# lmangani/duckdb-fastlane

Measured on AMD Instinct MI355X. Metric: decoded values/sec (lineitem_full SF100 full scan), higher is better.
Workload: dtype u8..u64 integer unpack -> int32/int64/string_t

## Files before the change

duckdb-fastlane_amd/csrc/fls_decode.hip:

```cpp
#include <hip/hip_runtime.h>

#include <algorithm>
#include <cstdlib>
#include <cstring>
#include <map>
#include <mutex>
#include <tuple>

#include "fls_alp.hpp"
#include "fls_decode.hpp"
#include "fls_format.hpp"
#include "fls_unpack.hpp"

#include "fls_decode_dev.hpp"

namespace fls {
using namespace dec;
namespace {

#ifndef FLS_WAVES_PER_SIMD
#define FLS_WAVES_PER_SIMD 4
#endif
template <bool RATING>
__global__ __launch_bounds__(256, FLS_WAVES_PER_SIMD) void decode_kernel(const DevChunk *__restrict__ chunks, uint32_t nchunks,
                                                        uint32_t *__restrict__ err, uint32_t p_bytes,
                                                        uint32_t v_bytes, uint32_t *__restrict__ queue,
                                                        const uint32_t *__restrict__ split, uint32_t npieces,
                                                        uint32_t flags) {
    extern __shared__ __attribute__((aligned(16))) uint8_t lds_raw[];
    const uint32_t shared_queue = flags & 1u, prio = (flags >> 1) & 3u;
    if (prio == 1) __builtin_amdgcn_s_setprio(1);
    else if (prio == 2) __builtin_amdgcn_s_setprio(2);
    else if (prio == 3) __builtin_amdgcn_s_setprio(3);
    const uint32_t w = uni(threadIdx.x >> 6);
    const uint32_t lp = (uint32_t)(size_t)((lu8 *)lds_raw + w * (p_bytes + v_bytes));
    const uint32_t lv = lp + p_bytes;
    const uint32_t stride = shared_queue ? 0u : gridDim.x * kWaves, first = blockIdx.x * kWaves + w;
    if (split && shared_queue) {
        const FLS_GLOBAL uint32_t *sp = gptr(split);
        const uint32_t nst = flags >> 8;
        for (;;) {
            uint32_t q = 0;
            if (__lane_id() == 0) q = atomicAdd(queue, 1u);
            q = uni(q);
            if (q >= nst + npieces) break;
            const uint32_t i = q < nst ? q : q + 1;
            decode_range(chunks, nchunks, uni(sp[i]), uni(sp[i + 1]), lp, lv, v_bytes, err);
        }
        return;
    }
    if (split) {
        const FLS_GLOBAL uint32_t *sp = gptr(split);
        decode_range(chunks, nchunks, uni(sp[first]), uni(sp[first + 1]), lp, lv, v_bytes, err);
        if (!queue) return;
        const FLS_GLOBAL uint32_t *pp = sp + stride + 1;
        for (;;) {
            uint32_t p = 0;
            if (__lane_id() == 0) p = atomicAdd(queue, 1u);
            p = uni(p);
            if (p >= npieces) break;
            decode_range(chunks, nchunks, uni(pp[p]), uni(pp[p + 1]), lp, lv, v_bytes, err);
        }
        return;
    }
    for (uint32_t ci = next_chunk(queue, UINT32_MAX, first, stride); ci < nchunks;
         ci = next_chunk(queue, ci, first, stride)) {
        const uint32_t nvec = gptr(chunks)[ci].nvec;
        if (nvec == 0) continue;
        decode_chunk(chunks + ci, lp, lv, v_bytes, err, nvec << 8);
    }
}

}

#ifdef FLS_WAVE_TRACE
extern "C" int fls_trace_reset(void) {
    const uint32_t z = 0;
    return hipMemcpyToSymbol(HIP_SYMBOL(g_trace_n), &z, sizeof(z)) == hipSuccess ? 0 : -1;
}
extern "C" int64_t fls_trace_read(void *dst, uint32_t cap) {
    uint32_t n = 0;
    if (hipDeviceSynchronize() != hipSuccess ||
        hipMemcpyFromSymbol(&n, HIP_SYMBOL(g_trace_n), sizeof(n)) != hipSuccess)
        return -1;
    const uint32_t k = std::min(std::min(n, cap), kTraceCap);
    if (k && hipMemcpyFromSymbol(dst, HIP_SYMBOL(g_trace), (size_t)k * sizeof(TraceRec)) != hipSuccess) return -1;
    return n;
}
#endif

namespace {
std::mutex g_occ_mu;
std::map<int, int> g_cus;
std::map<std::tuple<int, const void *, int, size_t>, int> g_occ;
}

int device_cus() {
    int dev = 0, cus = 256;
    if (hipGetDevice(&dev) != hipSuccess) return 256;
    {
        std::lock_guard<std::mutex> lk(g_occ_mu);
        if (auto it = g_cus.find(dev); it != g_cus.end()) return it->second;
    }
    if (hipDeviceGetAttribute(&cus, hipDeviceAttributeMultiprocessorCount, dev) != hipSuccess) return 256;
    std::lock_guard<std::mutex> lk(g_occ_mu);
    g_cus[dev] = cus;
    return cus;
}

int occupancy(const void *kernel, int block, size_t shmem) {
    int dev = 0, per_cu = 1;
    if (hipGetDevice(&dev) != hipSuccess) return 1;
    const auto key = std::make_tuple(dev, kernel, block, shmem);
    {
        std::lock_guard<std::mutex> lk(g_occ_mu);
        if (auto it = g_occ.find(key); it != g_occ.end()) return it->second;
    }
    if (hipOccupancyMaxActiveBlocksPerMultiprocessor(&per_cu, kernel, block, shmem) != hipSuccess) return 1;
    std::lock_guard<std::mutex> lk(g_occ_mu);
    g_occ[key] = per_cu;
    return per_cu;
}

int decode_grid_size(uint32_t shmem_per_block) {
    const int cus = device_cus();
    int per_cu = occupancy(reinterpret_cast<const void *>(decode_kernel<false>), 64 * kWaves, shmem_per_block);
    if (const char *e = getenv("FLS_BLOCKS_PER_CU")) per_cu = std::min(per_cu, std::max(1, atoi(e)));
    return cus * std::max(1, per_cu);
}

uint32_t decode_waves(const DecodeGeom &geom) {
    const uint32_t shmem = kWaves * (geom.p_bytes + geom.v_bytes);
    return (uint32_t)(geom.grid > 0 ? geom.grid : decode_grid_size(shmem)) * kWaves;
}

static inline uint64_t vec_cost(const DevChunk &d) { return 1024ull * d.ob + 128ull * d.max_w + 512; }

SplitPlan balanced_split(const DevChunk *h, uint32_t n, uint32_t nw, uint32_t static_pct, uint32_t pieces_per_wave,
                         std::vector<uint32_t> &pos) {
    uint64_t total = 0, nvecs = 0;
    for (uint32_t i = 0; i < n; ++i) {
        total += h[i].nvec * vec_cost(h[i]);
        nvecs += h[i].nvec;
    }
    SplitPlan plan;
    plan.waves = (uint32_t)std::min<uint64_t>(nw, (nvecs + kWaves - 1) / kWaves * kWaves);
    if (plan.waves == 0) plan.waves = kWaves;
    static_pct = std::min(static_pct, 100u);
    plan.pieces = static_pct < 100 ? plan.waves * std::max(1u, pieces_per_wave) : 0;
    const uint64_t stat = (uint64_t)((unsigned __int128)total * static_pct / 100);
    pos.clear();
    pos.reserve(plan.positions());
    uint64_t acc = 0;
    uint32_t i = 0;
    auto at = [&](uint64_t tgt) {
        while (i < n && acc + h[i].nvec * vec_cost(h[i]) <= tgt) {
            acc += h[i].nvec * vec_cost(h[i]);
            ++i;
        }
        pos.push_back(i < n ? (i << 7 | (uint32_t)((tgt - acc) / vec_cost(h[i]))) : n << 7);
    };
    for (uint32_t w = 0; w <= plan.waves; ++w) at((uint64_t)((unsigned __int128)stat * w / plan.waves));
    at(stat);
    for (uint32_t p = 1; p < plan.pieces; ++p) at(stat + (uint64_t)((unsigned __int128)(total - stat) * p / plan.pieces));
    if (plan.pieces) pos.push_back(n << 7);
    return plan;
}

SplitPlan guided_split(const DevChunk *h, uint32_t n, uint32_t nw, uint32_t factor, uint32_t min_vecs,
                       std::vector<uint32_t> &pos) {
    uint64_t total = 0;
    for (uint32_t i = 0; i < n; ++i) total += h[i].nvec * vec_cost(h[i]);
    factor = std::max(1u, factor);
    min_vecs = std::max(1u, min_vecs);
    nw = std::max<uint32_t>(nw, kWaves);
    std::vector<uint32_t> b;
    b.reserve(n + n / 4);
    uint64_t acc = 0;
    for (uint32_t i = 0; i < n; ++i) {
        const uint32_t nv = h[i].nvec;
        if (nv == 0) continue;
        const uint64_t vc = vec_cost(h[i]), cc = nv * vc;
        const uint64_t target = std::max<uint64_t>((total - acc) / ((uint64_t)factor * nw), (uint64_t)min_vecs * vc);
        uint32_t parts = 1;
        if (cc > target)
            parts = (uint32_t)std::min<uint64_t>((cc + target - 1) / target, (nv + min_vecs - 1) / min_vecs);
        for (uint32_t p = 0; p < parts; ++p) b.push_back(i << 7 | (uint32_t)((uint64_t)nv * p / parts));
        acc += cc;
    }
    const uint32_t items = (uint32_t)b.size();
    b.push_back(n << 7);
    SplitPlan plan;
    plan.guided = true;
    plan.waves = std::min<uint32_t>(nw, std::max<uint32_t>(kWaves, (items + kWaves - 1) / kWaves * kWaves));
    plan.pieces = items > plan.waves ? items - plan.waves : 0;
    pos.clear();
    pos.reserve(plan.positions());
    for (uint32_t w = 0; w <= plan.waves; ++w) pos.push_back(b[std::min(w, items)]);
    for (uint32_t p = 0; p <= plan.pieces; ++p) pos.push_back(b[std::min(plan.waves + p, items)]);
    return plan;
}

hipError_t launch_decode(const DevChunk *d_chunks, uint32_t nchunks, uint32_t *d_err, const DecodeGeom &geom,
                         hipStream_t stream, uint32_t *d_queue, const uint32_t *d_split, SplitPlan plan,
                         bool shared_queue, int prio) {
    if (nchunks == 0) return hipSuccess;
    const uint32_t shmem = kWaves * (geom.p_bytes + geom.v_bytes);
    int grid;
    if (d_split && shared_queue) {
        grid = std::min<int>(geom.grid > 0 ? geom.grid : decode_grid_size(shmem), (int)(plan.waves / kWaves));
    } else if (d_split) {
        grid = (int)(plan.waves / kWaves);
        if (!plan.pieces) d_queue = nullptr;
    } else {
        grid = std::min<int>(geom.grid > 0 ? geom.grid : decode_grid_size(shmem), (nchunks + kWaves - 1) / kWaves);
    }
    if (d_queue && !shared_queue) {
        const hipError_t e = hipMemsetAsync(d_queue, 0, sizeof(uint32_t), stream);
        if (e != hipSuccess) return e;
    }
    hipLaunchKernelGGL(rating_launch() ? decode_kernel<true> : decode_kernel<false>, dim3(grid), dim3(64 * kWaves), shmem,
                       stream, d_chunks, nchunks, d_err,
                       geom.p_bytes, geom.v_bytes, d_queue, d_split, plan.pieces,
                       (uint32_t)(shared_queue && d_queue) | (uint32_t)(prio & 3) << 1 |
                           (d_split && shared_queue ? plan.waves << 8 : 0u));
    return hipGetLastError();
}

bool &rating_launch() {
    static thread_local bool f = false;
    return f;
}

namespace {
__global__ __launch_bounds__(64) void probe_regions_kernel(const ProbeRegion *__restrict__ r, uint32_t n) {
    const uint32_t lane = threadIdx.x;
    for (uint32_t i = blockIdx.x; i < n; i += gridDim.x) {
        const uint64_t p = (uint64_t)r[i].out, nb = r[i].bytes >> 10;
        FLS_GLOBAL v4u *o = (FLS_GLOBAL v4u *)((uint64_t)uni((uint32_t)(p >> 32)) << 32 | (uint64_t)uni((uint32_t)p));
        const v4u z = {0u, 0u, 0u, 0u};
        for (uint64_t b = 0; b < nb; ++b) o[b * 64 + lane] = z;
    }
}
__global__ __launch_bounds__(256) void probe_fill_kernel(v4u *__restrict__ out) {
    ((FLS_GLOBAL v4u *)out)[(size_t)blockIdx.x * 256 + threadIdx.x] = v4u{0u, 0u, 0u, 0u};
}
}

hipError_t probe_placement(const ProbeRegion *d_regions, uint32_t nregions, uint8_t *const *bufs,
                           const uint64_t *buf_bytes, uint32_t nbuf, int reps, hipStream_t stream, float *chunk_ms,
                           float *fill_ms) {
    int dev = 0, cus = 256;
    hipError_t e = hipGetDevice(&dev);
    if (e != hipSuccess) return e;
    if (hipDeviceGetAttribute(&cus, hipDeviceAttributeMultiprocessorCount, dev) != hipSuccess) cus = 256;
    hipEvent_t a, b;
    if ((e = hipEventCreate(&a)) != hipSuccess) return e;
    if ((e = hipEventCreate(&b)) != hipSuccess) {
        hipEventDestroy(a);
        return e;
    }
    float best_c = 1e30f, best_f = 1e30f;
    for (int r = 0; r <= reps && e == hipSuccess; ++r) {
        float ms = 0;
        hipEventRecord(a, stream);
        hipLaunchKernelGGL(probe_regions_kernel, dim3(cus * 16), dim3(64), 0, stream, d_regions, nregions);
        hipEventRecord(b, stream);
        if ((e = hipEventSynchronize(b)) != hipSuccess) break;
        hipEventElapsedTime(&ms, a, b);
        if (r) best_c = std::min(best_c, ms);
        hipEventRecord(a, stream);
        for (uint32_t i = 0; i < nbuf; ++i)
            if (buf_bytes[i] >= 4096)
                hipLaunchKernelGGL(probe_fill_kernel, dim3((uint32_t)(buf_bytes[i] >> 12)), dim3(256), 0, stream,
                                   (v4u *)bufs[i]);
        hipEventRecord(b, stream);
        if ((e = hipEventSynchronize(b)) != hipSuccess) break;
// ... 13 lines not shown
```

duckdb-fastlane_amd/csrc/fls_decode.hpp:

```cpp
#pragma once
#include <hip/hip_runtime.h>

#include <cstdint>
#include <vector>

namespace fls {

struct DevChunk {
    const uint8_t *chunk;
    const uint8_t *dict;
    uint8_t *out;
    uint32_t nvec;
    uint32_t dict_count;
    uint32_t meta_off;
    uint32_t packed_off;
    uint32_t aux_off;
    uint8_t enc, T, vbits, ob;
    uint64_t heap_host;
    uint32_t heap_bytes;
    union {
        uint32_t vec_base;
        uint32_t max_w;
    };
};
static_assert(sizeof(DevChunk) == 64, "DevChunk is 64 B");

enum : uint32_t { KERR_DICT_CODE = 1, KERR_RUN_INDEX = 2, KERR_BAD_DESC = 4, KERR_FSST = 8 };
enum : uint32_t { KERR_LDS_BASE = 32 };

struct DecodeGeom {
    uint32_t p_bytes = 256, v_bytes = 0;
    int grid = 0;
};

struct SplitPlan {
    uint32_t waves = 0, pieces = 0;
    bool guided = false;
    size_t positions() const { return waves ? (size_t)waves + pieces + 2 : 0; }
};

hipError_t launch_decode(const DevChunk *d_chunks, uint32_t nchunks, uint32_t *d_err, const DecodeGeom &geom,
                         hipStream_t stream, uint32_t *d_queue = nullptr, const uint32_t *d_split = nullptr,
                         SplitPlan plan = SplitPlan(), bool shared_queue = false, int prio = 0);
uint32_t decode_waves(const DecodeGeom &geom);
SplitPlan balanced_split(const DevChunk *h, uint32_t n, uint32_t nw, uint32_t static_pct, uint32_t pieces_per_wave,
                         std::vector<uint32_t> &pos);
SplitPlan guided_split(const DevChunk *h, uint32_t n, uint32_t nw, uint32_t factor, uint32_t min_vecs,
                       std::vector<uint32_t> &pos);
enum : int {
    kFsstPlain = 1, kFsstTwoQ = 2, kFsstZeroFlush = 4, kFsstW6 = 8, kFsstCirc = 16, kFsstLenFromSym = 32, kFsstAbsLds = 64, kFsstEarlyGather = 128,
    kFsstDefault = kFsstW6 | kFsstZeroFlush | kFsstAbsLds,
    kFsstSegSparse = kFsstPlain,
    kFsstSegPackedLen = kFsstLenFromSym,
    kFsstSegWide = kFsstCirc,
    kFsstSegDouble = kFsstEarlyGather,
    kFsstSegBatch = 256,
    kFsstAblateRecords = 512, kFsstAblateFlush = 1024, kFsstAblateWrite = 2048,
    kFsstSegLean = 4096,
    kFsstSegD8 = 8192,
    kFsstSegLazy = 16384,
    kFsstSegW4 = 32768
};
struct FsstLaunch {
    int bytes_per_lane = 8;
    bool small = false;
    uint32_t *queue = nullptr;
    bool reset_queue = true;
    int waves_per_cu = 0;
    int grid_cus = 0;
    int variant = kFsstDefault;
    bool seg = false;
    int seg_cap = 4096;
};
hipError_t launch_fsst(const DevChunk *d_chunks, uint32_t nchunks, uint32_t nvecs, uint32_t *d_err,
                       hipStream_t stream, const FsstLaunch &how);
struct FusedLaunch {
    uint32_t fsst_per16 = 6;
    uint32_t piece = 2;
    bool halving = false;
    uint32_t fsst_static_pct = 0;
    bool static_first = true;
    int waves_per_cu = 0;
    int x = 0;
    uint32_t tail_chunks = 0, tail_split = 1;
};
hipError_t launch_fused(const DevChunk *d_main, uint32_t nmain, const DevChunk *d_fsst, uint32_t nfsst,
                        uint32_t nfvecs, bool small, uint32_t *d_err, const DecodeGeom &geom, hipStream_t stream,
                        uint32_t *d_queues, const FusedLaunch &how);
bool fsst_variant_built(int variant, bool seg, int bytes_per_lane);
bool fused_x_built(int x);
hipError_t launch_fsst_sp(const DevChunk *d_chunks, uint32_t nchunks, uint32_t nvecs, uint32_t *d_err,
                          hipStream_t stream);
struct DictVec {
    const uint8_t *packed;
    const uint8_t *tab;
    uint8_t *out;
    uint32_t base;
    uint32_t info;
};
static_assert(sizeof(DictVec) == 32, "DictVec is 32 B");
constexpr uint32_t kDictWgMaxEntries = 64;
inline bool dictstr_eligible(const DevChunk &c) {
    return c.enc == 3  && c.ob == 16 && c.T == 32 && c.nvec > 0 && c.dict_count >= 1 &&
           c.dict_count <= kDictWgMaxEntries && c.dict && ((uintptr_t)c.dict & 15) == 0 && ((uintptr_t)c.out & 15) == 0 &&
           (((uintptr_t)c.chunk + c.packed_off) & 15) == 0;
}
hipError_t launch_dictstr(const DictVec *d_vecs, uint32_t nvecs, uint32_t *d_err, hipStream_t stream);
int decode_grid_size(uint32_t shmem_per_block);
int device_cus();
int occupancy(const void *kernel, int block, size_t shmem);

bool &rating_launch();

struct ProbeRegion {
    uint8_t *out;
    uint64_t bytes;
};
hipError_t probe_placement(const ProbeRegion *d_regions, uint32_t nregions, uint8_t *const *bufs,
                           const uint64_t *buf_bytes, uint32_t nbuf, int reps, hipStream_t stream, float *chunk_ms,
                           float *fill_ms);
inline void chunk_lds_need(uint8_t enc, uint8_t T, uint8_t ob, uint32_t dict_count, uint32_t max_w,
                           uint32_t &p_bytes, uint32_t &v_bytes) {
    p_bytes = 128 * max_w + 128;
    v_bytes = 0;
    if (enc == 2  && T < 64) v_bytes = 128 * T;
    if (enc == 4 ) v_bytes = 2048;
    if (enc == 3 ) {
        const uint32_t d = dict_count * ob;
        v_bytes = 4096 + (d <= 4096 ? ((d + 15) & ~15u) : 0);
    }
}

}
```

duckdb-fastlane_amd/csrc/fls_decode_dev.hpp:

```cpp
#pragma once
#include <hip/hip_runtime.h>

#include <algorithm>
#include <cstdlib>
#include <cstring>

#include "fls_alp.hpp"
#include "fls_decode.hpp"
#include "fls_format.hpp"
#include "fls_unpack.hpp"

namespace fls {
namespace dec {
namespace {
using namespace dev;

constexpr int kWaves = 4;

using gv4 = const FLS_GLOBAL v4u;
using gu8 = const FLS_GLOBAL uint8_t;
using ov4 = FLS_GLOBAL v4u;
using ou8 = FLS_GLOBAL uint8_t;
using lv4 = FLS_LDS v4u;
using lu8 = FLS_LDS uint8_t;
// ... 437 lines not shown
template <>
struct AlpScale<32> {
    float fm, im;
    __device__ __forceinline__ AlpScale(uint32_t e, uint32_t f) : fm(kF10F[f]), im(kIF10F[e]) {}
    __device__ __forceinline__ uint32_t one(uint32_t d) const {
        return __float_as_uint((float)(int32_t)d * fm * im);
    }
    __device__ __forceinline__ v4u apply(v4u x) const { return mk4(one(x.x), one(x.y), one(x.z), one(x.w)); }
};

template <int T_>
struct PathAlp {
    static constexpr int T = T_;
    static constexpr uint32_t kMaxE = T_ == 64 ? kAlpMaxExpD : kAlpMaxExpF;
    using Aux = NoAux;
    gu8 *aux_base;
    uint32_t *err;
    __device__ __forceinline__ PathAlp(const DevChunk &c, const Lds &, uint32_t, uint32_t *e)
        : aux_base(gptr(c.chunk) + c.aux_off), err(e) {}
    __device__ __forceinline__ gu8 *aux_ptr(const DevChunk &, const VecInfo &) const { return nullptr; }
    template <bool FULL>
    __device__ __forceinline__ void vec(const Lds &s, const VecInfo &x, const Aux &, ou8 *out, uint32_t lane) const {
        const uint32_t exc = x.acount & 0xFFFF;
        const uint32_t e = min((x.acount >> 16) & 0xFF, kMaxE), f = min(x.acount >> 24, e);
        const AlpScale<T> sc(e, f);
        const uint32_t limit = x.nvals * (T / 8);
#pragma unroll
        for (uint32_t j = 0; j < T / 8; ++j) {
            const uint32_t ci = lane + 64 * j;
            const v4u v = sc.apply(add_base<T>(unpack_chunk<T>(s.P, x.W, ci), x.base));
            if (FULL) st16(out, 16 * ci, v);
            else store16<T / 8>(out, 16 * ci, limit, v);
            seq();
        }
        if (exc == 0) return;
        __builtin_amdgcn_s_waitcnt(0x0F70);
        gu8 *ea = aux_base + x.aoff;
        const FLS_GLOBAL uint16_t *pos = reinterpret_cast<const FLS_GLOBAL uint16_t *>(ea);
        gu8 *val = ea + ((2 * exc + 15) & ~15u);
        bool bad = false;
        for (uint32_t k = lane; k < exc; k += 64) {
            const uint32_t p = pos[k];
            if (p >= x.nvals) { bad = true; continue; }
            if (T == 64) {
                reinterpret_cast<FLS_GLOBAL uint64_t *>(out)[p] = reinterpret_cast<const FLS_GLOBAL uint64_t *>(val)[k];
            } else {
                reinterpret_cast<FLS_GLOBAL uint32_t *>(out)[p] = reinterpret_cast<const FLS_GLOBAL uint32_t *>(val)[k];
            }
        }
        if (bad) atomicOr(err, KERR_BAD_DESC);
    }
};

template <class Path, int L>
__device__ __attribute__((noinline)) void run_chunk(const DevChunk *chunk_generic, uint32_t lds_p, uint32_t lds_v,
                                                    uint32_t v_bytes, uint32_t *err_generic, uint32_t vrange) {
    const uint64_t cp = (uint64_t)chunk_generic;
    const FLS_GLOBAL DevChunk *cptr =
        (const FLS_GLOBAL DevChunk *)((uint64_t)uni((uint32_t)(cp >> 32)) << 32 | uni((uint32_t)cp));
    DevChunk c;
    {
        const FLS_GLOBAL v4u *q = reinterpret_cast<const FLS_GLOBAL v4u *>(cptr);
        v4u *d = reinterpret_cast<v4u *>(&c);
        d[0] = q[0];
        d[1] = q[1];
        d[2] = q[2];
        d[3] = q[3];
    }
    Lds s;
    s.P = (lv4 *)(size_t)uni(lds_p);
    s.V = (lu8 *)(size_t)uni(lds_v);
    s.v_bytes = uni(v_bytes);
    const uint64_t ep = (uint64_t)err_generic;
    uint32_t *err = (uint32_t *)((uint64_t)uni((uint32_t)(ep >> 32)) << 32 | uni((uint32_t)ep));
    const uint32_t lane = __lane_id();
    const Path path(c, s, lane, err);
    using Aux = typename Path::Aux;
    const uint32_t nvec = c.nvec;
    const uint32_t ob = c.ob;
    const ChunkMetas m = load_metas(c, lane);
    gv4 *packed = reinterpret_cast<gv4 *>(gptr(c.chunk) + c.packed_off);
    gv4 *dummy = reinterpret_cast<gv4 *>(gptr(c.chunk));
    ou8 *out = gptr(c.out);
    const uint32_t vb = uni(vrange) & 0xFF, ve = min(uni(vrange) >> 8, nvec);
    const uint32_t last_nvals = rl(m.nvbw, nvec - 1) & 0xFFFF;
    const uint32_t nfull = (ve == nvec && last_nvals != kVectorSize) ? ve - 1 : ve;

#ifdef FLS_PREFETCH2
    if (vb < ve) {
        v4u ra[L], rb[L];
        VecInfo xa = vec_info(m, vb);
        Aux aa, ab;
        aa.load(path.aux_ptr(c, xa), lane);
        prefetch<L, true>(packed + xa.poff16, 8 * xa.W, dummy, lane, ra);
        VecInfo xb = vec_info(m, min(vb + 1, ve - 1));
        ab.load(path.aux_ptr(c, xb), lane);
        prefetch<L, true>(packed + xb.poff16, 8 * xb.W, dummy, lane, rb);
        uint32_t v = vb;
        for (;;) {
            if (v >= nfull) break;
            wave_sync();
            stage<L>(s.P, ra, 8 * xa.W, lane);
            {
                const VecInfo xn = vec_info(m, min(v + 2, ve - 1));
                Aux an;
                an.load(path.aux_ptr(c, xn), lane);
                prefetch<L, true>(packed + xn.poff16, 8 * xn.W, dummy, lane, ra);
                wave_sync();
                path.template vec<true>(s, xa, aa, out + (size_t)v * kVectorSize * ob, lane);
                xa = xn;
                aa = an;
            }
            ++v;
            if (v >= nfull) break;
            wave_sync();
            stage<L>(s.P, rb, 8 * xb.W, lane);
            {
                const VecInfo xn = vec_info(m, min(v + 2, ve - 1));
                Aux an;
                an.load(path.aux_ptr(c, xn), lane);
                prefetch<L, true>(packed + xn.poff16, 8 * xn.W, dummy, lane, rb);
                wave_sync();
                path.template vec<true>(s, xb, ab, out + (size_t)v * kVectorSize * ob, lane);
                xb = xn;
                ab = an;
            }
            ++v;
        }
        if (nfull < ve) {
            wave_sync();
            const bool in_a = ((v - vb) & 1) == 0;
            if (in_a) stage<L>(s.P, ra, 8 * xa.W, lane);
            else stage<L>(s.P, rb, 8 * xb.W, lane);
            wave_sync();
            if (in_a) path.template vec<false>(s, xa, aa, out + (size_t)v * kVectorSize * ob, lane);
            else path.template vec<false>(s, xb, ab, out + (size_t)v * kVectorSize * ob, lane);
        }
    }
    return;
#endif
    v4u r[L];
    Aux aux, aux_next;
    VecInfo cur = vec_info(m, vb);
    aux.load(path.aux_ptr(c, cur), lane);
    prefetch<L>(packed + cur.poff16, 8 * cur.W, dummy, lane, r);
    uint32_t v = vb;
    if (vb < nfull) {
        stage<L>(s.P, r, 8 * cur.W, lane);
        VecInfo nxt = vec_info(m, vb + 1 < ve ? vb + 1 : vb);
        aux_next.load(path.aux_ptr(c, nxt), lane);
        prefetch<L>(packed + nxt.poff16, 8 * nxt.W, dummy, lane, r);
        wave_sync();
        path.template vec<true>(s, cur, aux, out + (size_t)vb * kVectorSize * ob, lane);
        cur = nxt;
        aux = aux_next;
        for (v = vb + 1; v < nfull; ++v) {
            wave_sync();
            stage<L>(s.P, r, 8 * cur.W, lane);
            nxt = vec_info(m, v + 1 < ve ? v + 1 : v);
            aux_next.load(path.aux_ptr(c, nxt), lane);
            prefetch<L>(packed + nxt.poff16, 8 * nxt.W, dummy, lane, r);
            wave_sync();
            path.template vec<true>(s, cur, aux, out + (size_t)v * kVectorSize * ob, lane);
            cur = nxt;
            aux = aux_next;
        }
    }
    if (nfull < ve) {
        wave_sync();
        stage<L>(s.P, r, 8 * cur.W, lane);
        wave_sync();
        path.template vec<false>(s, cur, aux, out + (size_t)v * kVectorSize * ob, lane);
    }
}

template <class Path, int L>
__device__ __forceinline__ void call_l(const DevChunk *c, uint32_t lp, uint32_t lv, uint32_t vb, uint32_t *err,
                                       uint32_t max_w, uint32_t vr) {
    if constexpr (L > 1) {
        if (max_w <= 4 * L) {
            call_l<Path, L / 2>(c, lp, lv, vb, err, max_w, vr);
            return;
        }
    }
    run_chunk<Path, L>(c, lp, lv, vb, err, vr);
}
template <class Path>
__device__ __forceinline__ void call(const DevChunk *c, uint32_t lp, uint32_t lv, uint32_t vb, uint32_t *err,
                                     uint32_t max_w, uint32_t vr) {
    call_l<Path, Path::T / 8>(c, lp, lv, vb, err, max_w, vr);
}

template <int OB>
__device__ __forceinline__ void call_dict(const DevChunk *c, uint32_t lp, uint32_t lv, uint32_t vb, uint32_t *err,
                                          uint32_t dict_count, uint32_t max_w, uint32_t vr) {
    if (dict_count * OB + 4096 <= vb) call<PathDict<OB, true>>(c, lp, lv, vb, err, max_w, vr);
    else call<PathDict<OB, false>>(c, lp, lv, vb, err, max_w, vr);
}

__device__ __forceinline__ uint32_t next_chunk(uint32_t *queue, uint32_t prev, uint32_t first, uint32_t stride) {
    if (prev == UINT32_MAX && stride) return first;
    if (!queue) return prev + stride;
    uint32_t ci = 0;
    if (__lane_id() == 0) ci = atomicAdd(queue, 1u);
    return stride + uni(ci);
}

#ifdef FLS_WAVE_TRACE
struct TraceRec {
    uint64_t t0, t1;
    uint32_t wave, vr, hw_id, xcc_id, shape, max_w;
};
constexpr uint32_t kTraceCap = 1u << 20;
__device__ TraceRec g_trace[kTraceCap];
__device__ uint32_t g_trace_n;
#endif

__device__ __forceinline__ void decode_chunk_body(const DevChunk *cg, uint32_t lp, uint32_t lv, uint32_t v_bytes,
                                                  uint32_t *err, uint32_t vr);
__device__ __forceinline__ void decode_chunk(const DevChunk *cg, uint32_t lp, uint32_t lv, uint32_t v_bytes,
                                             uint32_t *err, uint32_t vr) {
#ifdef FLS_WAVE_TRACE
    const uint64_t t0 = wall_clock64();
    decode_chunk_body(cg, lp, lv, v_bytes, err, vr);
    const uint64_t t1 = wall_clock64();
    if (__lane_id() == 0) {
        const uint32_t i = atomicAdd(&g_trace_n, 1u);
        if (i < kTraceCap) {
            const FLS_GLOBAL DevChunk *c = gptr(cg);
            TraceRec &r = g_trace[i];
            r.t0 = t0;
            r.t1 = t1;
            r.wave = blockIdx.x * kWaves + (threadIdx.x >> 6);
            r.vr = vr;
            r.hw_id = __builtin_amdgcn_s_getreg((31 << 11) | 4);
// ... 5 lines not shown
#else
    decode_chunk_body(cg, lp, lv, v_bytes, err, vr);
#endif
}
__device__ __forceinline__ void decode_chunk_body(const DevChunk *cg, uint32_t lp, uint32_t lv, uint32_t v_bytes,
                                                  uint32_t *err, uint32_t vr) {
    const FLS_GLOBAL DevChunk *c = gptr(cg);
    const uint32_t dc = c->dict_count, mw = c->max_w;
    const uint32_t enc = c->enc, T = c->T, ob = c->ob;
    switch (enc) {
    case ENC_FFOR:
        switch (T) {
        case 64: call<PathFfor<64>>(cg, lp, lv, v_bytes, err, mw, vr); break;
        case 32: call<PathFfor<32>>(cg, lp, lv, v_bytes, err, mw, vr); break;
        case 16: call<PathFfor<16>>(cg, lp, lv, v_bytes, err, mw, vr); break;
        default: call<PathFfor<8>>(cg, lp, lv, v_bytes, err, mw, vr); break;
        }
        break;
    case ENC_DELTA:
        switch (T) {
        case 64: call<PathDelta64>(cg, lp, lv, v_bytes, err, mw, vr); break;
        case 32: call<PathDeltaSmall<32>>(cg, lp, lv, v_bytes, err, mw, vr); break;
        case 16: call<PathDeltaSmall<16>>(cg, lp, lv, v_bytes, err, mw, vr); break;
        default: call<PathDeltaSmall<8>>(cg, lp, lv, v_bytes, err, mw, vr); break;
        }
        break;
    case ENC_DICT:
        switch (ob) {
        case 16: call_dict<16>(cg, lp, lv, v_bytes, err, dc, mw, vr); break;
        case 8: call_dict<8>(cg, lp, lv, v_bytes, err, dc, mw, vr); break;
        case 4: call_dict<4>(cg, lp, lv, v_bytes, err, dc, mw, vr); break;
        case 2: call_dict<2>(cg, lp, lv, v_bytes, err, dc, mw, vr); break;
        default: call_dict<1>(cg, lp, lv, v_bytes, err, dc, mw, vr); break;
        }
        break;
    case ENC_ALP:
        if (T == 64) call<PathAlp<64>>(cg, lp, lv, v_bytes, err, mw, vr);
        else call<PathAlp<32>>(cg, lp, lv, v_bytes, err, mw, vr);
        break;
    case ENC_RLE:
        switch (ob) {
        case 8: call<PathRle<8>>(cg, lp, lv, v_bytes, err, mw, vr); break;
        case 4: call<PathRle<4>>(cg, lp, lv, v_bytes, err, mw, vr); break;
        case 2: call<PathRle<2>>(cg, lp, lv, v_bytes, err, mw, vr); break;
        default: call<PathRle<1>>(cg, lp, lv, v_bytes, err, mw, vr); break;
        }
        break;
    default:
        if ((threadIdx.x & 63) == 0) atomicOr(err, KERR_BAD_DESC);
        break;
    }
}

__device__ __forceinline__ void decode_range(const DevChunk *chunks, uint32_t nchunks, uint32_t s0, uint32_t s1,
                                             uint32_t lp, uint32_t lv, uint32_t v_bytes, uint32_t *err) {
    const uint32_t ce = min(s1 >> 7, nchunks), vend = s1 & 127;
    uint32_t vb = s0 & 127;
    for (uint32_t ci = s0 >> 7; ci < ce || (ci == ce && ci < nchunks && vb < vend); ++ci, vb = 0) {
        const uint32_t nvec = gptr(chunks)[ci].nvec;
        const uint32_t ve = min(ci == ce ? vend : nvec, nvec);
        if (vb < ve) decode_chunk(chunks + ci, lp, lv, v_bytes, err, vb | ve << 8);
    }
}

}
}
}
```

duckdb-fastlane_amd/csrc/fls_fsst.hip:

```cpp
#include <hip/hip_runtime.h>

#include <algorithm>
#include <cstdio>
#include <cstdlib>

#include "fls_decode.hpp"
#include "fls_decode_dev.hpp"
#include "fls_format.hpp"
#include "fls_unpack.hpp"

namespace fls {
namespace {
using namespace dev;

using gv4 = const FLS_GLOBAL v4u;
using gu8 = const FLS_GLOBAL uint8_t;
using ov4 = FLS_GLOBAL v4u;
using lv4 = FLS_LDS v4u;
using lu8 = FLS_LDS uint8_t;
using lu16 = FLS_LDS uint16_t;
using lu32 = FLS_LDS uint32_t;
using lu64 = FLS_LDS uint64_t;

__device__ __forceinline__ uint32_t rl(uint32_t x, uint32_t l) { return __builtin_amdgcn_readlane(x, l); }
// ... 951 lines not shown
    const uint32_t shmem = K == Kind::Seg ? SegLds<SMALL, X>::kWave : CpLds<SMALL>::kWave;
    auto kern = fsst_kernel<K, SMALL, QUEUE, X>;
    static const bool lds_at_zero = [kern] {
        hipFuncAttributes a{};
        return hipFuncGetAttributes(&a, reinterpret_cast<const void *>(kern)) == hipSuccess && a.sharedSizeBytes == 0;
    }();
    if (!lds_at_zero) {
        fprintf(stderr, "fsst_kernel: static LDS present or attributes unavailable; cannot address LDS from 0\n");
        return hipErrorInvalidDeviceFunction;
    }
    int cus = device_cus(), per_cu = occupancy(reinterpret_cast<const void *>(kern), 64, shmem);
    if (how.grid_cus > 0) cus = std::min(cus, how.grid_cus);
    const int full = cus * std::max(1, per_cu);
    int wpc = how.waves_per_cu;
    if (const char *e = getenv("FLS_FSST_WPC"); e && wpc == 0) wpc = std::max(0, atoi(e));
    const int grid = std::min<int>(wpc > 0 ? cus * std::min(wpc, per_cu) : full, (int)nvecs);
    uint32_t piece = std::max<uint32_t>(1, std::min<uint32_t>(16, nvecs / (4u * (uint32_t)full)));
    if (const char *e = getenv("FLS_FSST_PIECE")) piece = (uint32_t)std::max(1, std::min(64, atoi(e)));
    if (how.queue && how.reset_queue) {
        const hipError_t e = hipMemsetAsync(how.queue, 0, sizeof(uint32_t), stream);
        if (e != hipSuccess) return e;
    }
    if (getenv("FLS_DEBUG"))
        fprintf(stderr, "DEBUG: fsst_kernel<%d,%s%s>: %d blocks of 1 wave (%d per CU, %u B LDS), %u vectors%s\n",
                K == Kind::Seg ? 16 : 8, SMALL ? "small" : "any", K == Kind::Seg ? ",seg" : "", grid, per_cu, shmem,
                nvecs, how.queue ? " (piece queue)" : "");
    hipLaunchKernelGGL(kern, dim3(grid), dim3(64), shmem, stream, d_chunks, nchunks, nvecs, d_err, how.queue, piece);
    return hipGetLastError();
}
template <Kind K, int X = 0>
hipError_t launch_kind2(const DevChunk *d, uint32_t nchunks, uint32_t nvecs, uint32_t *err, hipStream_t stream,
                        const FsstLaunch &how) {
    if (how.queue) return how.small ? launch_kind<K, true, true, X>(d, nchunks, nvecs, err, stream, how)
                                    : launch_kind<K, false, true, X>(d, nchunks, nvecs, err, stream, how);
    return how.small ? launch_kind<K, true, false, X>(d, nchunks, nvecs, err, stream, how)
                     : launch_kind<K, false, false, X>(d, nchunks, nvecs, err, stream, how);
}

template <bool SMALL, int X>
__device__ __attribute__((noinline)) void fused_fsst_part(const DevChunk *fchunks, uint32_t nfsst, uint32_t nfvecs,
                                                          uint32_t item0, uint32_t item1, uint32_t *queue,
                                                          uint32_t piece, uint32_t qbase, uint32_t *err) {
    fsst_range<Kind::Seg, SMALL, true, X>(fchunks, nfsst, nfvecs, uni(item0), uni(item1), uni_ptr(queue), uni(piece),
                                          (lu8 *)(size_t)0, err, uni(qbase));
}

template <bool SMALL, int X = 0, bool RATING = false>
__global__ __launch_bounds__(64, 4) void fused_kernel(const DevChunk *__restrict__ mchunks, uint32_t nmain,
                                                      const DevChunk *__restrict__ fchunks, uint32_t nfsst,
                                                      uint32_t nfvecs, uint32_t *__restrict__ err,
                                                      uint32_t *__restrict__ queues, uint32_t p_bytes,
                                                      uint32_t v_bytes, uint32_t piece, uint32_t fsst_per16,
                                                      uint32_t fsst_static, uint32_t nf_waves, uint32_t nwhole,
                                                      uint32_t tsplit) {
    extern __shared__ __attribute__((aligned(16))) uint8_t lds_raw[];
    if ((uint32_t)(size_t)lds_raw != 0u) {
        if (threadIdx.x == 0) atomicOr(err, KERR_LDS_BASE);
        return;
    }
    const uint32_t b = blockIdx.x, k = fsst_per16, grp = b >> 4, r = b & 15;
    const bool fsst_first = r < k;
    const uint32_t nitems = nwhole + (nmain - nwhole) * tsplit;
    auto main_part = [&](bool first) {
        uint32_t it = first ? grp * (16 - k) + (r - k) : 0u;
        for (;; first = false) {
            if (!first) {
                if (__lane_id() == 0) it = atomicAdd(queues, 1u);
                it = uni(it);
            }
            if (it >= nitems) {
                if (first) continue;
                break;
            }
            uint32_t ci = it, p = 0;
            if (it >= nwhole) {
                ci = nwhole + (it - nwhole) / tsplit;
                p = (it - nwhole) % tsplit;
            }
            const uint32_t nvec = gptr(mchunks)[ci].nvec;
            const uint32_t vb = it >= nwhole ? nvec * p / tsplit : 0u, ve = it >= nwhole ? nvec * (p + 1) / tsplit : nvec;
            if (vb < ve) dec::decode_chunk(mchunks + ci, 0u, p_bytes, v_bytes, err, vb | ve << 8);
        }
    };
    auto fsst_part = [&](bool first) {
        uint32_t i0 = 0, i1 = 0;
        if (first) {
            const uint32_t f = grp * k + r;
            i0 = (uint32_t)((uint64_t)fsst_static * f / nf_waves);
            i1 = (uint32_t)((uint64_t)fsst_static * (f + 1) / nf_waves);
        }
        if (nfsst) fused_fsst_part<SMALL, X>(fchunks, nfsst, nfvecs, i0, i1, queues + 1, piece, fsst_static, err);
        wave_sync();
    };
    const bool stat = nf_waves != 0;
    if (fsst_first) {
        fsst_part(stat);
        main_part(false);
    } else {
        main_part(stat);
        fsst_part(false);
    }
}

template <bool SMALL, int X = 0>
hipError_t launch_fused_t(const DevChunk *d_main, uint32_t nmain, const DevChunk *d_fsst, uint32_t nfsst,
                          uint32_t nfvecs, uint32_t *d_err, const DecodeGeom &geom, hipStream_t stream,
                          uint32_t *d_queues, const FusedLaunch &how) {
    auto kern = rating_launch() ? fused_kernel<SMALL, X, true> : fused_kernel<SMALL, X, false>;
    const uint32_t shmem = std::max<uint32_t>(geom.p_bytes + geom.v_bytes, SegLds<SMALL>::kWave);
    static const bool lds_at_zero = [] {
        auto zero = [](auto k) {
            hipFuncAttributes a{};
            return hipFuncGetAttributes(&a, reinterpret_cast<const void *>(k)) == hipSuccess && a.sharedSizeBytes == 0;
        };
        return zero(fused_kernel<SMALL, X, false>) && zero(fused_kernel<SMALL, X, true>);
    }();
    if (!lds_at_zero) return hipErrorInvalidDeviceFunction;
    const int cus = device_cus();
    int per_cu = occupancy(reinterpret_cast<const void *>(kern), 64, shmem);
    if (how.waves_per_cu > 0) per_cu = std::min(per_cu, how.waves_per_cu);
    const int grid = cus * std::max(1, per_cu);
    const uint32_t k = std::min(16u, how.fsst_per16);
    uint32_t nf = 0;
    for (int bb = 0; bb < grid; ++bb) nf += (uint32_t)(bb & 15) < k;
    const uint32_t nm = (uint32_t)grid - nf;
    const bool stat = how.static_first;
    const uint32_t tsplit = std::max(1u, std::min(64u, how.tail_split));
    const uint32_t nwhole = tsplit > 1 ? nmain - std::min(nmain, how.tail_chunks) : nmain;
    const uint32_t nitems = nwhole + (nmain - nwhole) * tsplit;
    const uint32_t fstat = stat && nf ? (uint32_t)((uint64_t)nfvecs * std::min(100u, how.fsst_static_pct) / 100) : 0u;
    hipError_t e = hipMemsetD32Async((hipDeviceptr_t)d_queues, stat ? std::min(nm, nitems) : 0u, 1, stream);
    if (e == hipSuccess) e = hipMemsetD32Async((hipDeviceptr_t)(d_queues + 1), 0, 1, stream);
    if (e != hipSuccess) return e;
    if (getenv("FLS_DEBUG"))
        fprintf(stderr, "DEBUG: fused_kernel<%s>: %d blocks of 1 wave (%d per CU, %u B LDS), %u main chunks, %u FSST "
                        "vectors in pieces of %u, %u of 16 waves FSST first\n",
                SMALL ? "small" : "any", grid, per_cu, shmem, nmain, nfvecs, how.piece, how.fsst_per16);
    hipLaunchKernelGGL(kern, dim3(grid), dim3(64), shmem, stream, d_main, nmain, d_fsst, nfsst, nfvecs, d_err,
                       d_queues, geom.p_bytes, geom.v_bytes, std::max(1u, std::min(64u, how.piece)) | (how.halving ? kHalving : 0u),
                       k, fstat, stat ? std::max(1u, nf) : 0u, nwhole, tsplit);
    return hipGetLastError();
}

constexpr uint32_t kSpIncap = 1536;
constexpr uint32_t kSpOutcap = 2560;
constexpr uint32_t kSpSym = 0, kSpLen = 2048, kSpDL = 2304, kSpCL = kSpDL + 1024, kSpIn = kSpCL + 1024;
constexpr uint32_t kSpOut = kSpIn + kSpIncap + 16;
constexpr uint32_t kSpWave = kSpOut + kSpOutcap + 16;
static_assert(kSpIncap >= 128 * 8 + 128 && kSpIncap >= 255 + 16 && kSpOutcap >= 255 + 16, "SP ring sizes");
static_assert(kSpIn % 16 == 0 && kSpOut % 16 == 0 && kSpWave % 16 == 0, "SP LDS layout alignment");

struct SpWave {
    const lu64 *sym;
    const lu8 *len;
    lu8 *DL, *CL, *IN, *OUT;
};

__device__ __forceinline__ void unpack_u8(const SpWave &w, gu8 *packed, uint32_t W, uint32_t base, uint32_t nvals,
                                          lu8 *dst, uint32_t lane) {
    lv4 *P = reinterpret_cast<lv4 *>(w.IN);
    stage_packed(P, packed, W, lane);
#pragma unroll
    for (uint32_t j = 0; j < 4; ++j) {
        const uint32_t ci = lane + 64 * j;
        const v4u v = length_chunk(P, W, base, nvals, ci);
        reinterpret_cast<lu32 *>(dst)[ci] = (v.x & 255) | (v.y & 255) << 8 | (v.z & 255) << 16 | (v.w & 255) << 24;
    }
    wave_sync();
}

__device__ __forceinline__ uint32_t wave_max(uint32_t x) {
    x = max(x, (uint32_t)__builtin_amdgcn_update_dpp(0u, x, 0x111, 0xf, 0xf, false));
    x = max(x, (uint32_t)__builtin_amdgcn_update_dpp(0u, x, 0x112, 0xf, 0xf, false));
    x = max(x, (uint32_t)__builtin_amdgcn_update_dpp(0u, x, 0x114, 0xf, 0xf, false));
    x = max(x, (uint32_t)__builtin_amdgcn_update_dpp(0u, x, 0x118, 0xf, 0xf, false));
    x = max(x, (uint32_t)__builtin_amdgcn_update_dpp(0u, x, 0x142, 0xa, 0xf, false));
    x = max(x, (uint32_t)__builtin_amdgcn_update_dpp(0u, x, 0x143, 0xc, 0xf, false));
    return rl(x, 63);
}

__device__ __forceinline__ bool sp_decode(const SpWave &w, uint32_t cb, uint32_t cl, uint32_t wp, uint32_t dl,
                                          uint32_t maxcl) {
    const lu32 *in32 = reinterpret_cast<const lu32 *>(w.IN);
    lu64 *o64 = reinterpret_cast<lu64 *>(w.OUT);
    constexpr uint32_t kLastQ = (kSpOutcap + 16) / 8 - 1;
    const uint32_t ce = cb + cl;
    uint32_t q = wp >> 3, bits = 8 * (wp & 7), pos = 0;
    uint64_t acc = 0;
    bool lit = false;
    for (uint32_t it = 0; it < maxcl; it += 4) {
        const uint32_t c = cb + it;
        const uint32_t x = __builtin_amdgcn_alignbyte(in32[(c >> 2) + 1], in32[c >> 2], c & 3);
        const uint32_t nk = c < ce ? min(ce - c, 4u) : 0u;
// ... 259 lines not shown
```

duckdb-fastlane_amd/csrc/flsgpu.hip:

```cpp
#include <fcntl.h>
#include <hip/hip_runtime.h>
#include <hip/hip_ext.h>
#include <sys/mman.h>
#include <sys/stat.h>
#include <unistd.h>

#include "fls_engine.hpp"

using namespace fls;
using namespace fls::engine;

FLS_ENGINE_BEGIN

static StrT make_string_t(const char *p, uint32_t n) {
    StrT s;
    memset(&s, 0, sizeof(s));
    s.len = n;
    if (n <= 12) {
        memcpy(s.data, p, n);
    } else {
        memcpy(s.data, p, 4);
        memcpy(s.data + 4, &p, sizeof(p));
    }
    return s;
// ... 489 lines not shown
    if (const char *e = getenv("FLS_OVERLAP_GUIDED")) o.guided = atoi(e) != 0;
    return o;
}

int fsst_config_check(int64_t policy) {
    int variant = kFsstDefault;
    const char *fv = getenv("FLS_FSST_VARIANT");
    if (fv) {
        char *end = nullptr;
        const long v = strtol(fv, &end, 10);
        if (end == fv || *end != 0 || v < 0 || v > 0x7FFFFFFF)
            return fail(FLS_ERR_CONFIG, "FLS_FSST_VARIANT=%s is not a variant number", fv);
        variant = (int)v;
    }
    if (const char *fx = getenv("FLS_FUSED_X")) {
        char *end = nullptr;
        const long x = strtol(fx, &end, 10);
        if (end == fx || *end != 0 || x < 0 || x > 0x7FFFFFFF || !fused_x_built((int)x))
            return fail(FLS_ERR_CONFIG,
                        "FLS_FUSED_X=%s is not in this build: the product library holds the default fused kernel "
                        "only; experiments need FLS_LIB=libflsgpu_lab.so (make lab) -- unset FLS_FUSED_X",
                        fx);
    }
    const int bpl = (policy & POLICY_FSST16) ? 16 : 8;
    if (!fsst_variant_built(variant, true, bpl) || !fsst_variant_built(variant, false, bpl))
        return fail(FLS_ERR_CONFIG,
                    "FSST kernel variant %d (%d bytes per lane) is not in this build: the product library holds the "
                    "default kernels only; experiments need FLS_LIB=libflsgpu_lab.so (make lab)%s",
                    variant, bpl, fv ? " -- unset FLS_FSST_VARIANT" : "");
    return 0;
}

struct FusedCfg {
    int mode = 1;
    uint32_t min_vecs_per_cu = 0;
    bool per16_set = false;
    bool variant = false;
    FusedLaunch how;
};
static FusedCfg fused_cfg() {
    FusedCfg f;
    if (const char *e = getenv("FLS_FUSED")) f.mode = std::min(2, std::max(0, atoi(e) == 1 ? 2 : atoi(e)));
    if (const char *e = getenv("FLS_FUSED_FSST16")) {
        f.how.fsst_per16 = (uint32_t)std::min(16, std::max(0, atoi(e)));
        f.per16_set = true;
    }
    if (const char *e = getenv("FLS_FUSED_PIECE")) f.how.piece = (uint32_t)std::min(64, std::max(1, atoi(e)));
    if (const char *e = getenv("FLS_FUSED_WPC")) f.how.waves_per_cu = std::max(0, atoi(e));
    if (const char *e = getenv("FLS_FUSED_STATIC_PCT")) f.how.fsst_static_pct = (uint32_t)std::min(100, std::max(0, atoi(e)));
    if (const char *e = getenv("FLS_FUSED_STATIC_FIRST")) f.how.static_first = atoi(e) != 0;
    if (const char *e = getenv("FLS_FUSED_HALVING")) f.how.halving = atoi(e) != 0;
    if (const char *e = getenv("FLS_FUSED_TAIL")) f.how.tail_chunks = (uint32_t)std::max(0, atoi(e));
    if (const char *e = getenv("FLS_FUSED_TAIL_SPLIT")) f.how.tail_split = (uint32_t)std::min(64, std::max(1, atoi(e)));
    if (const char *e = getenv("FLS_FUSED_X")) f.how.x = atoi(e);
    if (const char *e = getenv("FLS_FUSED_MIN_VECS_PER_CU")) f.min_vecs_per_cu = (uint32_t)std::max(0, atoi(e));
    if (const char *e = getenv("FLS_FSST_VARIANT"))
        if (atoi(e) != kFsstDefault) f.variant = true;
    return f;
}

template <class LaunchGroup>
static hipError_t launch_cu_split(const DevChunk *d_chunks, uint32_t nmain, const FsstCounts &fc, uint32_t *d_err,
                           const DecodeGeom &geom, hipStream_t stream, uint32_t *d_queue, SideStream *side,
                           const OverlapSplit &ov, int cus, const FsstLaunch (&how)[kFsstGroups],
                           LaunchGroup &launch_group) {
    const int m = ov.cu_split;
    uint32_t mask_a[8] = {}, mask_b[8] = {};
    int na = 0, nb = 0;
    for (int i = 0; i < std::min(cus, 256); ++i) {
        if (i % 32 < m) {
            mask_a[i / 32] |= 1u << (i % 32);
            ++na;
        } else {
            mask_b[i / 32] |= 1u << (i % 32);
            ++nb;
        }
    }
    if (na == 0 || nb == 0) return hipErrorInvalidValue;
    if (side->cu_m != m) {
        side->release_cu();
        hipError_t e = hipExtStreamCreateWithCUMask(&side->cu_a, 8, mask_a);
        if (e == hipSuccess) e = hipExtStreamCreateWithCUMask(&side->cu_b, 8, mask_b);
        if (e == hipSuccess) e = hipEventCreateWithFlags(&side->join_a, hipEventDisableTiming);
        if (e == hipSuccess) e = hipEventCreateWithFlags(&side->join_b, hipEventDisableTiming);
        if (e != hipSuccess) {
            side->release_cu();
            return e;
        }
        side->cu_m = m;
    }
    const uint32_t shmem = 4 * (geom.p_bytes + geom.v_bytes);
    const int bpc = std::max(1, (geom.grid > 0 ? geom.grid : decode_grid_size(shmem)) / std::max(1, cus));
    DecodeGeom ga = geom, gb = geom;
    ga.grid = na * bpc;
    gb.grid = nb * bpc;
    FsstLaunch ha[kFsstGroups], hb[kFsstGroups];
    for (int g = 0; g < kFsstGroups; ++g) {
        ha[g] = hb[g] = how[g];
        ha[g].queue = hb[g].queue = d_queue + 1 + g;
        ha[g].reset_queue = hb[g].reset_queue = false;
        ha[g].grid_cus = na;
        hb[g].grid_cus = nb;
    }
    hipError_t e = hipMemsetAsync(d_queue, 0, kQueueWords * sizeof(uint32_t), stream);
    if (e == hipSuccess) e = hipEventRecord(side->fork, stream);
    if (e == hipSuccess) e = hipStreamWaitEvent(side->cu_a, side->fork, 0);
// ... 1660 lines not shown
```

Before: 482.5 billion.

## Add burst multi-vector prefetch pipeline to chunk decode for small-width paths

```diff
diff --git a/duckdb-fastlane_amd/csrc/fls_decode.hip b/duckdb-fastlane_amd/csrc/fls_decode.hip
--- a/duckdb-fastlane_amd/csrc/fls_decode.hip
+++ b/duckdb-fastlane_amd/csrc/fls_decode.hip
@@ -28,7 +28,7 @@
                                                         const uint32_t *__restrict__ split, uint32_t npieces,
                                                         uint32_t flags) {
     extern __shared__ __attribute__((aligned(16))) uint8_t lds_raw[];
-    const uint32_t shared_queue = flags & 1u, prio = (flags >> 1) & 3u;
+    const uint32_t shared_queue = flags & 1u, prio = (flags >> 1) & 3u, burst = (flags >> 3) & 15u;
     if (prio == 1) __builtin_amdgcn_s_setprio(1);
     else if (prio == 2) __builtin_amdgcn_s_setprio(2);
     else if (prio == 3) __builtin_amdgcn_s_setprio(3);
@@ -45,13 +45,13 @@
             q = uni(q);
             if (q >= nst + npieces) break;
             const uint32_t i = q < nst ? q : q + 1;
-            decode_range(chunks, nchunks, uni(sp[i]), uni(sp[i + 1]), lp, lv, v_bytes, err);
+            decode_range(chunks, nchunks, uni(sp[i]), uni(sp[i + 1]), lp, lv, v_bytes, err, burst);
         }
         return;
     }
     if (split) {
         const FLS_GLOBAL uint32_t *sp = gptr(split);
-        decode_range(chunks, nchunks, uni(sp[first]), uni(sp[first + 1]), lp, lv, v_bytes, err);
+        decode_range(chunks, nchunks, uni(sp[first]), uni(sp[first + 1]), lp, lv, v_bytes, err, burst);
         if (!queue) return;
         const FLS_GLOBAL uint32_t *pp = sp + stride + 1;
         for (;;) {
@@ -59,7 +59,7 @@
             if (__lane_id() == 0) p = atomicAdd(queue, 1u);
             p = uni(p);
             if (p >= npieces) break;
-            decode_range(chunks, nchunks, uni(pp[p]), uni(pp[p + 1]), lp, lv, v_bytes, err);
+            decode_range(chunks, nchunks, uni(pp[p]), uni(pp[p + 1]), lp, lv, v_bytes, err, burst);
         }
         return;
     }
@@ -67,7 +67,7 @@
          ci = next_chunk(queue, ci, first, stride)) {
         const uint32_t nvec = gptr(chunks)[ci].nvec;
         if (nvec == 0) continue;
-        decode_chunk(chunks + ci, lp, lv, v_bytes, err, nvec << 8);
+        decode_chunk(chunks + ci, lp, lv, v_bytes, err, nvec << 8 | burst_bits(burst));
     }
 }
 
@@ -127,6 +127,12 @@
     int per_cu = occupancy(reinterpret_cast<const void *>(decode_kernel<false>), 64 * kWaves, shmem_per_block);
     if (const char *e = getenv("FLS_BLOCKS_PER_CU")) per_cu = std::min(per_cu, std::max(1, atoi(e)));
     return cus * std::max(1, per_cu);
+}
+
+uint32_t burst_cap() {
+    uint32_t cap = 4;
+    if (const char *e = getenv("FLS_BURST")) cap = (uint32_t)std::min(8, std::max(0, atoi(e)));
+    return cap;
 }
 
 uint32_t decode_waves(const DecodeGeom &geom) {
@@ -222,7 +228,7 @@
     hipLaunchKernelGGL(rating_launch() ? decode_kernel<true> : decode_kernel<false>, dim3(grid), dim3(64 * kWaves), shmem,
                        stream, d_chunks, nchunks, d_err,
                        geom.p_bytes, geom.v_bytes, d_queue, d_split, plan.pieces,
-                       (uint32_t)(shared_queue && d_queue) | (uint32_t)(prio & 3) << 1 |
+                       (uint32_t)(shared_queue && d_queue) | (uint32_t)(prio & 3) << 1 | burst_cap() << 3 |
                            (d_split && shared_queue ? plan.waves << 8 : 0u));
     return hipGetLastError();
 }
diff --git a/duckdb-fastlane_amd/csrc/fls_decode.hpp b/duckdb-fastlane_amd/csrc/fls_decode.hpp
--- a/duckdb-fastlane_amd/csrc/fls_decode.hpp
+++ b/duckdb-fastlane_amd/csrc/fls_decode.hpp
@@ -43,6 +43,7 @@
                          hipStream_t stream, uint32_t *d_queue = nullptr, const uint32_t *d_split = nullptr,
                          SplitPlan plan = SplitPlan(), bool shared_queue = false, int prio = 0);
 uint32_t decode_waves(const DecodeGeom &geom);
+uint32_t burst_cap();
 SplitPlan balanced_split(const DevChunk *h, uint32_t n, uint32_t nw, uint32_t static_pct, uint32_t pieces_per_wave,
                          std::vector<uint32_t> &pos);
 SplitPlan guided_split(const DevChunk *h, uint32_t n, uint32_t nw, uint32_t factor, uint32_t min_vecs,
@@ -83,6 +84,7 @@
     int waves_per_cu = 0;
     int x = 0;
     uint32_t tail_chunks = 0, tail_split = 1;
+    uint32_t burst = 4;
 };
 hipError_t launch_fused(const DevChunk *d_main, uint32_t nmain, const DevChunk *d_fsst, uint32_t nfsst,
                         uint32_t nfvecs, bool small, uint32_t *d_err, const DecodeGeom &geom, hipStream_t stream,
diff --git a/duckdb-fastlane_amd/csrc/fls_decode_dev.hpp b/duckdb-fastlane_amd/csrc/fls_decode_dev.hpp
--- a/duckdb-fastlane_amd/csrc/fls_decode_dev.hpp
+++ b/duckdb-fastlane_amd/csrc/fls_decode_dev.hpp
@@ -513,7 +513,23 @@
     }
 };
 
-template <class Path, int L>
+template <int L1, int L2, int L4>
+struct BurstMaxIs {
+    static constexpr int l1 = L1, l2 = L2, l4 = L4;
+};
+template <class Path> struct BurstMax : BurstMaxIs<4, 2, 1> {};
+template <> struct BurstMax<PathFfor<16>> : BurstMaxIs<4, 4, 1> {};
+template <> struct BurstMax<PathFfor<32>> : BurstMaxIs<4, 4, 2> {};
+template <> struct BurstMax<PathAlp<64>> : BurstMaxIs<4, 1, 1> {};
+template <> struct BurstMax<PathDeltaSmall<32>> : BurstMaxIs<4, 1, 1> {};
+template <> struct BurstMax<PathRle<4>> : BurstMaxIs<4, 1, 1> {};
+template <> struct BurstMax<PathDict<16, true>> : BurstMaxIs<2, 1, 1> {};
+template <> struct BurstMax<PathDict<8, false>> : BurstMaxIs<2, 1, 1> {};
+template <> struct BurstMax<PathDelta64> : BurstMaxIs<1, 1, 1> {};
+template <> struct BurstMax<PathDict<16, false>> : BurstMaxIs<1, 1, 1> {};
+template <> struct BurstMax<PathRle<8>> : BurstMaxIs<1, 1, 1> {};
+
+template <class Path, int L, int G = 1>
 __device__ __attribute__((noinline)) void run_chunk(const DevChunk *chunk_generic, uint32_t lds_p, uint32_t lds_v,
                                                     uint32_t v_bytes, uint32_t *err_generic, uint32_t vrange) {
     const uint64_t cp = (uint64_t)chunk_generic;
@@ -543,7 +559,7 @@
     gv4 *packed = reinterpret_cast<gv4 *>(gptr(c.chunk) + c.packed_off);
     gv4 *dummy = reinterpret_cast<gv4 *>(gptr(c.chunk));
     ou8 *out = gptr(c.out);
-    const uint32_t vb = uni(vrange) & 0xFF, ve = min(uni(vrange) >> 8, nvec);
+    const uint32_t vb = uni(vrange) & 0xFF, ve = min((uni(vrange) >> 8) & 0xFF, nvec);
     const uint32_t last_nvals = rl(m.nvbw, nvec - 1) & 0xFFFF;
     const uint32_t nfull = (ve == nvec && last_nvals != kVectorSize) ? ve - 1 : ve;
 
@@ -600,22 +616,71 @@
     }
     return;
 #endif
+    uint32_t v0 = vb;
+    if constexpr (G > 1) {
+        if (vb + 1 + G <= nfull) {
+            v4u rb[G][L];
+            Aux ab[G], a_last;
+            auto issue = [&](uint32_t vs) {
+#pragma unroll
+                for (int g = 0; g < G; ++g) {
+                    const VecInfo x = vec_info(m, vs + g);
+                    (g == G - 1 ? a_last : ab[g]).load(path.aux_ptr(c, x), lane);
+                }
+#pragma unroll
+                for (int g = 0; g < G; ++g) {
+                    const VecInfo x = vec_info(m, vs + g);
+                    prefetch<L, true>(packed + x.poff16, 8 * x.W, dummy, lane, rb[g]);
+                }
+            };
+            {
+                v4u r0[L];
+                Aux a0;
+                const VecInfo x = vec_info(m, vb);
+                a0.load(path.aux_ptr(c, x), lane);
+                prefetch<L>(packed + x.poff16, 8 * x.W, dummy, lane, r0);
+                stage<L>(s.P, r0, 8 * x.W, lane);
+                issue(vb + 1);
+                wave_sync();
+                path.template vec<true>(s, x, a0, out + (size_t)vb * kVectorSize * ob, lane);
+                ab[G - 1] = a_last;
+            }
+            uint32_t v = vb + 1;
+            for (;;) {
+                const bool more = v + 2 * G <= nfull;
+#pragma unroll
+                for (int g = 0; g < G; ++g) {
+                    const VecInfo x = vec_info(m, v + g);
+                    wave_sync();
+                    stage<L>(s.P, rb[g], 8 * x.W, lane);
+                    if (g == G - 1 && more) issue(v + G);
+                    wave_sync();
+                    path.template vec<true>(s, x, ab[g], out + (size_t)(v + g) * kVectorSize * ob, lane);
+                }
+                ab[G - 1] = a_last;
+                v += G;
+                if (!more) break;
+            }
+            v0 = v;
+        }
+    }
+    if (v0 >= ve) return;
     v4u r[L];
     Aux aux, aux_next;
-    VecInfo cur = vec_info(m, vb);
+    VecInfo cur = vec_info(m, v0);
     aux.load(path.aux_ptr(c, cur), lane);
     prefetch<L>(packed + cur.poff16, 8 * cur.W, dummy, lane, r);
-    uint32_t v = vb;
-    if (vb < nfull) {
+    uint32_t v = v0;
+    if (v0 < nfull) {
         stage<L>(s.P, r, 8 * cur.W, lane);
-        VecInfo nxt = vec_info(m, vb + 1 < ve ? vb + 1 : vb);
+        VecInfo nxt = vec_info(m, v0 + 1 < ve ? v0 + 1 : v0);
         aux_next.load(path.aux_ptr(c, nxt), lane);
         prefetch<L>(packed + nxt.poff16, 8 * nxt.W, dummy, lane, r);
         wave_sync();
-        path.template vec<true>(s, cur, aux, out + (size_t)vb * kVectorSize * ob, lane);
+        path.template vec<true>(s, cur, aux, out + (size_t)v0 * kVectorSize * ob, lane);
         cur = nxt;
         aux = aux_next;
-        for (v = vb + 1; v < nfull; ++v) {
+        for (v = v0 + 1; v < nfull; ++v) {
             wave_sync();
             stage<L>(s.P, r, 8 * cur.W, lane);
             nxt = vec_info(m, v + 1 < ve ? v + 1 : v);
@@ -642,6 +707,22 @@
         if (max_w <= 4 * L) {
             call_l<Path, L / 2>(c, lp, lv, vb, err, max_w, vr);
             return;
+        }
+    }
+    const uint32_t cap = vr >> 16;
+    if constexpr (L <= 4) {
+        constexpr int gmax = L == 1 ? BurstMax<Path>::l1 : L == 2 ? BurstMax<Path>::l2 : BurstMax<Path>::l4;
+        if constexpr (gmax >= 4) {
+            if (cap >= 4) {
+                run_chunk<Path, L, 4>(c, lp, lv, vb, err, vr);
+                return;
+            }
+        }
+        if constexpr (gmax >= 2) {
+            if (cap >= 2) {
+                run_chunk<Path, L, 2>(c, lp, lv, vb, err, vr);
+                return;
+            }
         }
     }
     run_chunk<Path, L>(c, lp, lv, vb, err, vr);
@@ -753,17 +834,20 @@
     }
 }
 
+__device__ __forceinline__ uint32_t burst_bits(uint32_t cap) { return min(cap, 8u) << 16; }
+
 __device__ __forceinline__ void decode_range(const DevChunk *chunks, uint32_t nchunks, uint32_t s0, uint32_t s1,
-                                             uint32_t lp, uint32_t lv, uint32_t v_bytes, uint32_t *err) {
+                                             uint32_t lp, uint32_t lv, uint32_t v_bytes, uint32_t *err,
+                                             uint32_t burst) {
     const uint32_t ce = min(s1 >> 7, nchunks), vend = s1 & 127;
     uint32_t vb = s0 & 127;
     for (uint32_t ci = s0 >> 7; ci < ce || (ci == ce && ci < nchunks && vb < vend); ++ci, vb = 0) {
         const uint32_t nvec = gptr(chunks)[ci].nvec;
         const uint32_t ve = min(ci == ce ? vend : nvec, nvec);
-        if (vb < ve) decode_chunk(chunks + ci, lp, lv, v_bytes, err, vb | ve << 8);
-    }
-}
-
-}
-}
-}
+        if (vb < ve) decode_chunk(chunks + ci, lp, lv, v_bytes, err, vb | ve << 8 | burst_bits(burst));
+    }
+}
+
+}
+}
+}
diff --git a/duckdb-fastlane_amd/csrc/fls_fsst.hip b/duckdb-fastlane_amd/csrc/fls_fsst.hip
--- a/duckdb-fastlane_amd/csrc/fls_fsst.hip
+++ b/duckdb-fastlane_amd/csrc/fls_fsst.hip
@@ -1027,7 +1027,7 @@
                                                       uint32_t *__restrict__ queues, uint32_t p_bytes,
                                                       uint32_t v_bytes, uint32_t piece, uint32_t fsst_per16,
                                                       uint32_t fsst_static, uint32_t nf_waves, uint32_t nwhole,
-                                                      uint32_t tsplit) {
+                                                      uint32_t tsplit, uint32_t burst) {
     extern __shared__ __attribute__((aligned(16))) uint8_t lds_raw[];
     if ((uint32_t)(size_t)lds_raw != 0u) {
         if (threadIdx.x == 0) atomicOr(err, KERR_LDS_BASE);
@@ -1054,7 +1054,7 @@
             }
             const uint32_t nvec = gptr(mchunks)[ci].nvec;
             const uint32_t vb = it >= nwhole ? nvec * p / tsplit : 0u, ve = it >= nwhole ? nvec * (p + 1) / tsplit : nvec;
-            if (vb < ve) dec::decode_chunk(mchunks + ci, 0u, p_bytes, v_bytes, err, vb | ve << 8);
+            if (vb < ve) dec::decode_chunk(mchunks + ci, 0u, p_bytes, v_bytes, err, vb | ve << 8 | dec::burst_bits(burst));
         }
     };
     auto fsst_part = [&](bool first) {
@@ -1113,7 +1113,7 @@
                 SMALL ? "small" : "any", grid, per_cu, shmem, nmain, nfvecs, how.piece, how.fsst_per16);
     hipLaunchKernelGGL(kern, dim3(grid), dim3(64), shmem, stream, d_main, nmain, d_fsst, nfsst, nfvecs, d_err,
                        d_queues, geom.p_bytes, geom.v_bytes, std::max(1u, std::min(64u, how.piece)) | (how.halving ? kHalving : 0u),
-                       k, fstat, stat ? std::max(1u, nf) : 0u, nwhole, tsplit);
+                       k, fstat, stat ? std::max(1u, nf) : 0u, nwhole, tsplit, std::min(8u, how.burst));
     return hipGetLastError();
 }
 
diff --git a/duckdb-fastlane_amd/csrc/flsgpu.hip b/duckdb-fastlane_amd/csrc/flsgpu.hip
--- a/duckdb-fastlane_amd/csrc/flsgpu.hip
+++ b/duckdb-fastlane_amd/csrc/flsgpu.hip
@@ -565,6 +565,7 @@
     if (const char *e = getenv("FLS_FUSED_HALVING")) f.how.halving = atoi(e) != 0;
     if (const char *e = getenv("FLS_FUSED_TAIL")) f.how.tail_chunks = (uint32_t)std::max(0, atoi(e));
     if (const char *e = getenv("FLS_FUSED_TAIL_SPLIT")) f.how.tail_split = (uint32_t)std::min(64, std::max(1, atoi(e)));
+    f.how.burst = burst_cap();
     if (const char *e = getenv("FLS_FUSED_X")) f.how.x = atoi(e);
     if (const char *e = getenv("FLS_FUSED_MIN_VECS_PER_CU")) f.min_vecs_per_cu = (uint32_t)std::max(0, atoi(e));
     if (const char *e = getenv("FLS_FSST_VARIANT"))
```

Result: no change. 487.2 billion, median of 6 (+1.0%).
